# SebastianBitsch/SRGAN-ST

Measured on AMD Instinct MI355X. Metric: HR images/sec (96px x4, B=16/GPU) G+D+ST-loss step, higher is better.
Workload: dtype f32; 1 GPU; srgan_x4_hr96_b16_G+D+ST-loss step: adv+mse+st, D updated every step (train.py:116-164; BASELINE metric); global_batch=16, hr=96, lr=24, parallelism=dp1, hip_graph=True, d_update_interval=1, d_sr_forward=run: all three discriminator forwards of train.py:136,155,158

## Files before the change

### include/srganst.h

```cpp
#ifndef SRGANST_H
#define SRGANST_H
#include <stdint.h>
#ifdef __cplusplus
extern "C" {
#endif

const char* sst_last_error(void);
int sst_version(void);
const char* sst_arch(void);
int sst_clear_error(void);
int sst_reload_env(void);

int sst_st_loss_workspace(int B, int H, int W, int64_t* partial_floats);
int sst_st_loss_fwd(const float* sr, const float* gt, float* loss, float* gS, float* partials,
                    unsigned* counter, int B, int H, int W, float sigma, float rho, int normalize,
                    void* stream);
int sst_st_loss_bwd(const float* sr, const float* gS, float* dsr, const float* scale_dev,
                    float scale_host, int accumulate, int B, int H, int W, float sigma, float rho,
                    void* stream);
int sst_st_maps_workspace(int B, int H, int W, int64_t* tile_floats);
int sst_st_maps(const float* x, const float* gt, float* Sx, float* Sgt, float* Fx, float* Fgt, float* d, float* tile_sums,
                int B, int H, int W, float sigma, float rho, int normalize, void* stream);
int sst_st_pixel_loss_fwd(const float* sr, const float* gt, float* loss, float* gS, float* partials, unsigned* counter,
                          float* pix_loss, float* pix_partials, int pix_mode, int B, int H, int W, float sigma, float rho,
// ... 106 lines not shown
int sst_conv_fwd_resin(const float* x, const float* y2, const float* ones, const float* bn_scale, const float* bn_shift,
                       float* h_out, const float* wp, float* y, const float* bias, float* stats, float* stats_cnt,
                       int B, int H, int W, int Cin, int Cout, int ksize, void* stream);
int sst_conv_dgrad_fused(const float* g, const float* y2, const float* cA, const float* cB, const float* cC,
                         const float* in_scale, const float* in_shift, const float* in_slope, float in_slope_const,
                         int in_act, float* dy_out, const float* wp, float* out, const float* residual,
                         const float* epi_y, const float* epi_scale, const float* epi_shift, const float* epi_slope,
                         float epi_slope_const, int epi_act, float* epi_partial, int B, int H, int W, int Cin, int Cout,
                         int ksize, void* stream);
int sst_conv_wgrad_chunks2(int B, int H, int W, int Cin, int Cout, int ksize, int stride, int njobs);
int sst_conv_wgrad_groups_ok(int B, int H, int W, int Cin, int Cout, int ksize, int stride, int grp_images);
int sst_conv_wgrad_grp(const float* x, const float* dy, float* slab, float* dw, const float* in_scale,
                   const float* in_shift, const float* in_slope, float in_slope_const, int in_act,
                   int B, int H, int W, int Cin, int Cout, int stride, int ksize, int accumulate,
                       int grp_images, void* stream);
int sst_conv_wgrad_pending_reduce(int B, int H, int W, int Cin, int Cout, int ksize, int stride, int has_in_scale, int in_act);
int sst_wgrad_reduce_multi(const void* jobs, int njobs, void* stream);
int sst_wgrad_c3_supported(int C, int ksize);
int64_t sst_wgrad_c3_slab_floats(int B, int H, int W, int C);
int sst_wgrad_c3(const float* big, const float* small, float* slab, float* dw, const float* in_slope,
                 float in_slope_const, int in_act, int kind, int B, int H, int W, int C, int accumulate,
                 void* stream);

int64_t sst_conv9_c3_packed_floats(int Cout_eff);
int sst_conv9_c3_pack(const float* w, float* wp, int Cout, int Cin, int mode, void* stream);
int sst_conv9_c3_fwd(const float* x, const float* wp, float* y, const float* bias, int B, int H, int W,
                     int Cout, void* stream);
int64_t sst_conv9_to3_packed_floats(int C);
int sst_conv9_to3_pack(const float* w, float* wp, int C, void* stream);
int sst_conv9_to3_fwd(const float* x, const float* wp, float* y, float* y_pre, const float* bias,
// ... 151 lines not shown
```

### srgan-st_amd/csrc/bn_elem.hip

```cpp
#include "common.h"
#include <cstdlib>

typedef float f32x4 __attribute__((ext_vector_type(4)));

namespace {

constexpr int NT = 256;

__global__ __launch_bounds__(NT) void bn_finalize_kernel(const float* __restrict__ stats, const float* __restrict__ cnt,
                                                         int ntiles, int C, const float* __restrict__ gamma,
                                                         const float* __restrict__ beta, float* __restrict__ run_mean,
                                                         float* __restrict__ run_var, float* __restrict__ mean_out,
                                                         float* __restrict__ rstd_out, float* __restrict__ scale,
                                                         float* __restrict__ shift, float eps, float momentum, int groups) {
  __shared__ float red[2][NT / 64];
  const int c = blockIdx.x;
  for (int grp = 0; grp < groups; ++grp, stats += (size_t)ntiles * 2 * C, cnt += ntiles, mean_out += C, rstd_out += C, scale += C,
           shift += C) {
  constexpr int KT = 4;
  float ts[KT], tm[KT], tn[KT];
  float s = 0.f, n = 0.f;
#pragma unroll
  for (int k = 0; k < KT; ++k) {
    const int t = threadIdx.x + k * NT;
// ... 426 lines not shown
      if (scale) {
        ksc = *reinterpret_cast<const f32x4*>(scale + c);
        ksh = *reinterpret_cast<const f32x4*>(shift + c);
      }
      if (cA) {
        kA = *reinterpret_cast<const f32x4*>(cA + c);
        kB = *reinterpret_cast<const f32x4*>(cB + c);
        kC = *reinterpret_cast<const f32x4*>(cC + c);
      }
    }
#pragma unroll
    for (int j = 0; j < 4; ++j) {
      float gz = gv[j];
      if (act) {
        const float z = scale ? fmaf(yv[j], ksc[j], ksh[j]) : yv[j];
        gz = z > 0.f ? gz : gz * slope;
      }
      o[j] = cA ? fmaf(kA[j], gz, fmaf(kB[j], yv[j], kC[j])) : gz;
    }
    if (uW == 0) {
      reinterpret_cast<f32x4*>(dy)[i] = o;
    } else {
      const int64_t r = i / c4n;
      const int X = (int)(r % uW);
      const int64_t t = r / uW;
      const int Y = (int)(t % uH);
      const int64_t b = t / uH;
      float* d = dy + (((b * (uH >> 1) + (Y >> 1)) * (uW >> 1) + (X >> 1)) * (int64_t)(4 * C)) + 2 * (Y & 1) + (X & 1);
#pragma unroll
      for (int j = 0; j < 4; ++j) d[4 * (c + j)] = o[j];
    }
// ... 248 lines not shown
```

### srgan-st_amd/csrc/common.h

```cpp
#pragma once
#include <hip/hip_runtime.h>
#include <cstdarg>
#include <cstdio>
#include <cstdint>

#define SST_API extern "C" __attribute__((visibility("default")))

enum : int {
  SST_OK = 0,
  SST_ERR_ARG = -1,
  SST_ERR_UNSUPPORTED = -2,
  SST_ERR_HIP = -3,
};

int sst_set_error(int code, const char* fmt, ...);

#define SST_REQUIRE(cond, ...)                                   \
  do {                                                           \
    if (!(cond)) return sst_set_error(SST_ERR_ARG, __VA_ARGS__); \
  } while (0)

#define SST_LAUNCH_CHECK(name)                                                                   \
  do {                                                                                           \
    hipError_t e_ = hipGetLastError();                                                           \
    if (e_ != hipSuccess) return sst_set_error(SST_ERR_HIP, "%s: %s", name, hipGetErrorString(e_)); \
  } while (0)

const char* sst_env(const char* name);

static inline hipStream_t sst_stream(void* s) { return reinterpret_cast<hipStream_t>(s); }

__device__ __forceinline__ float wave_sum(float v) {
#pragma unroll
  for (int o = 32; o > 0; o >>= 1) v += __shfl_xor(v, o, 64);
  return v;
}

template <int NT>
__device__ __forceinline__ float block_sum(float v, float* red) {
  v = wave_sum(v);
  const int wid = threadIdx.x >> 6, lane = threadIdx.x & 63;
  __syncthreads();
  if (lane == 0) red[wid] = v;
  __syncthreads();
  float t = 0.f;
// ... 83 lines not shown
```

### srgan-st_amd/csrc/conv_fwd.hip

```cpp
#include "conv_common.h"
#include <cstdlib>
#include "conv_epilogue.h"

int sst_launch_conv_fwd2(const Conv3Args& a, int stride, hipStream_t st);
int sst_launch_conv_band(const Conv3Args& a, int R, hipStream_t st, const BandAcc* acc);
int sst_conv_band_rows(int B, int H, int W, int Cin, int Cout, int ksize, int stride);

namespace {

constexpr int BIG_MIN_TILES = 2048;
inline bool use_big_tiles(const Conv3Args& a, int ksize) {
  if (ksize != 3 || a.Cout < 64 || a.in2 || a.side_out) return false;
  if (a.out_mode != OUT_NHWC && a.out_mode != OUT_SHUFFLE && a.out_mode != OUT_STRIDE2) return false;
  if (const char* e = sst_env("SST_CONV_BIG")) return atoi(e) != 0;
  const long tiles = (long)a.B * ((a.Ho + 7) / 8) * ((a.Wo + 7) / 8) * ((a.Cout + 63) / 64);
  return tiles >= BIG_MIN_TILES;
}

template <int KS, int S>
__device__ __forceinline__ void conv_fwd_body(const Conv3Args& a, const int bx, const int by) {
  const int KK = a.ksy * a.ksx;
  constexpr int PW = (TWO - 1) * S + KS, PH = (THO - 1) * S + KS, NP = PW * PH;
  constexpr int LDS_FLOATS = (NP * LDSC > 4 * 32 * 33) ? NP * LDSC : 4 * 32 * 33;
  __shared__ __attribute__((aligned(16))) float lds[LDS_FLOATS];
// ... 454 lines not shown
        if (bias) v += *reinterpret_cast<const f32x4*>(bias + c);
        *reinterpret_cast<f32x4*>(ps + li * C3F_OST + c) = v;
      }
    const int b = t / (H * tpr), rem = t - b * (H * tpr);
    const int oy = rem / tpr, x0 = (rem - oy * tpr) << 5;
    float* const yp = y + (((size_t)b * H + oy) * W + x0) * Cout;
#pragma unroll
    for (int i = 0; i < 8; ++i) {
      const int idx = lane + 64 * i, px = idx >> 4, c4 = (idx & 15) * 4;
      *reinterpret_cast<f32x4*>(yp + (size_t)px * Cout + c4) = *reinterpret_cast<const f32x4*>(ps + px * C3F_OST + c4);
    }
  }
}

typedef float f32x4c __attribute__((ext_vector_type(4)));
__global__ __launch_bounds__(CONV_NT) void conv3_to3_kernel(const float* __restrict__ x, const float* __restrict__ wp,
                                                            float* __restrict__ y, int B, int H, int W, int nmt, int nsp) {
  extern __shared__ __attribute__((aligned(16))) float pl_all[];
  const int wave = __builtin_amdgcn_readfirstlane(threadIdx.x >> 6), lane = threadIdx.x & 63;
  const int seg = blockIdx.x * 4 + wave;
  if (seg >= B * H * nsp) return;
  const int row = seg / nsp, Ws = W / nsp, xb = (seg - row * nsp) * Ws;
  const int b = row / H, oy = row - b * H;
  const int lm = lane & 15, lg = lane >> 4;
  float* const pl = pl_all + (size_t)wave * nmt * 16 * 12;
  float bw[3][4][4];
  {
    const int tx = lm / 3, ci = lm - tx * 3;
#pragma unroll
    for (int ty = 0; ty < 3; ++ty)
#pragma unroll
      for (int q = 0; q < 4; ++q)
#pragma unroll
        for (int t = 0; t < 4; ++t) {
          const int co = 16 * q + 4 * lg + t, tap = ty * 3 + tx;
          bw[ty][q][t] = lm < 9 ? wp[(size_t)(tap * 8 + (co >> 3)) * 256 + (((co & 7) >> 2) * 32 + ci) * 4 + (co & 3)] : 0.f;
        }
  }
  auto load_tile = [&](int mt, f32x4c (&a)[3][4]) {
    const int xp = xb + mt * 16 + lm - 1;
#pragma unroll
    for (int ty = 0; ty < 3; ++ty) {
      const int iy = oy - 1 + ty;
      const bool ok = (unsigned)iy < (unsigned)H && (unsigned)xp < (unsigned)W;
      const float* src = x + (((size_t)b * H + (ok ? iy : 0)) * W + (ok ? xp : 0)) * 64 + 4 * lg;
#pragma unroll
      for (int q = 0; q < 4; ++q) {
        const f32x4c v = *reinterpret_cast<const f32x4c*>(src + 16 * q);
        a[ty][q] = ok ? v : f32x4c{0.f, 0.f, 0.f, 0.f};
      }
    }
  };
  f32x4c ac[3][4], an[3][4];
  load_tile(0, ac);
  for (int mt = 0; mt < nmt; ++mt) {
    if (mt + 1 < nmt) load_tile(mt + 1, an);
    f32x4c acc = {0.f, 0.f, 0.f, 0.f};
#pragma unroll
    for (int ty = 0; ty < 3; ++ty)
#pragma unroll
      for (int q = 0; q < 4; ++q)
#pragma unroll
        for (int t = 0; t < 4; ++t) acc = __builtin_amdgcn_mfma_f32_16x16x4f32(ac[ty][q][t], bw[ty][q][t], acc, 0, 0, 0);
    if (lm < 9) {
#pragma unroll
      for (int r = 0; r < 4; ++r) pl[(mt * 16 + 4 * lg + r) * 12 + lm] = acc[r];
    }
#pragma unroll
    for (int ty = 0; ty < 3; ++ty)
#pragma unroll
      for (int q = 0; q < 4; ++q) ac[ty][q] = an[ty][q];
  }
  float* const out = y + (((size_t)b * H + oy) * W + xb) * 3;
  for (int i = lane; i < 3 * Ws; i += 64) {
    const int xo = i / 3, ci = i - xo * 3;
    out[i] = (pl[xo * 12 + ci] + pl[(xo + 1) * 12 + 3 + ci]) + pl[(xo + 2) * 12 + 6 + ci];
  }
}

__global__ void pack_conv_kernel(const float* __restrict__ w, float* __restrict__ wp, int Cout, int Cin, int KK,
                                 int mode, int64_t total) {
  const int O = mode ? Cin : Cout, I = mode ? Cout : Cin;
  const int ncb = (I + 63) / 64;
  const int64_t base = packed_floats_base(O, I, KK);
  for (int64_t idx = blockIdx.x * (int64_t)blockDim.x + threadIdx.x; idx < total; idx += (int64_t)gridDim.x * blockDim.x) {
    if (idx >= base) {
      const int64_t q = idx - base;
      const int l = (q >> 2) & 63, tap = (q >> 10) % 9;
      const int o = (int)((q >> 10) / 9) * 16 + (l & 15), i = ((q >> 8) & 3) * 16 + (l >> 4) * 4 + (q & 3);
      wp[idx] = mode == 0 ? w[((size_t)o * Cin + i) * KK + tap] : w[((size_t)i * Cin + o) * KK + (KK - 1 - tap)];
      continue;
    }
// ... 365 lines not shown
  Conv3Args a{};
  conv_shape_args(a, B, H, W, Cin, Cout, ksize, stride);
  a.out_mode = out_mode;
  a.in2 = fused_in ? reinterpret_cast<const float*>(1) : nullptr;
  return conv_fwd_select(a, ksize, stride, 0).name;
}

SST_API int sst_conv_fwd(const float* x, const float* wp, float* y, float* y_pre, const float* bias, const float* in_scale,
                         const float* in_shift, const float* in_slope, float in_slope_const, int in_act,
                         const float* residual, float* stats, float* stats_cnt, int out_mode, int B, int H, int W, int Cin,
                         int Cout, int ksize, int stride, void* stream) {
  return conv_fwd_impl(x, wp, y, y_pre, bias, in_scale, in_shift, in_slope, in_slope_const, in_act, residual, stats, stats_cnt,
                       out_mode, B, H, W, Cin, Cout, ksize, stride, nullptr, nullptr, nullptr, nullptr, 0.f, 0, nullptr, stream);
}

SST_API int sst_conv_dgrad_bwdstats(const float* x, const float* wp, float* y, const float* residual, const float* epi_y,
                                    const float* epi_scale, const float* epi_shift, const float* epi_slope,
                                    float epi_slope_const, int epi_act, float* epi_partial, int B, int H, int W, int Cin,
                                    int Cout, int ksize, void* stream) {
  SST_REQUIRE(epi_y && epi_partial, "sst_conv_dgrad_bwdstats: epi_y / epi_partial");
  return conv_fwd_impl(x, wp, y, nullptr, nullptr, nullptr, nullptr, nullptr, 0.f, ACT_NONE, residual, nullptr, nullptr, OUT_NHWC,
                       B, H, W, Cin, Cout, ksize, 1, epi_y, epi_scale, epi_shift, epi_slope, epi_slope_const, epi_act, epi_partial,
                       stream);
}

SST_API int sst_conv_dgrad_fused(const float* g, const float* y2, const float* cA, const float* cB, const float* cC,
                                 const float* in_scale, const float* in_shift, const float* in_slope, float in_slope_const,
                                 int in_act, float* dy_out, const float* wp, float* out, const float* residual,
                                 const float* epi_y, const float* epi_scale, const float* epi_shift, const float* epi_slope,
                                 float epi_slope_const, int epi_act, float* epi_partial, int B, int H, int W, int Cin, int Cout,
// ... 200 lines not shown
```

### srgan-st_amd/csrc/conv_wgrad.hip

```cpp
#include "conv_common.h"
#include <cstring>
#include <cstdlib>

namespace {

constexpr int SUB = 64;
constexpr int WLD = 64 + 4;

struct WgJob {
  const float* x; const float* dy; float* slab; float* dw;
  const float* in_scale; const float* in_shift; const float* in_slope;
  float in_slope_const; int in_act;
};

constexpr int WG_TAB_MAX = 40;
struct WgJobTab { WgJob j[WG_TAB_MAX]; };

struct WgradArgs {
  int grouped;
  int nchunk;
  const float* x;
  const float* dy;
  float* slab;
  const float* in_scale;
// ... 366 lines not shown
    __syncthreads();
    if (pl == 0 && cob + co < Cout) {
      float* out = slab + (size_t)blockIdx.x * 9 * Cout * 3;
#pragma unroll
      for (int k = 0; k < 27; ++k) {
        const float t = ((acc[k] + red[0][co][k]) + red[1][co][k]) + red[2][co][k];
        const int ky = k / 9, kx = (k % 9) / 3, ci = k % 3;
        out[((size_t)(ky * 3 + kx) * Cout + cob + co) * 3 + ci] = t;
      }
    }
  }
}
constexpr int C3M_ROW = 104;
constexpr int C3M_WAVE = 3 * C3M_ROW + 96;
constexpr int C3M_TPW = 4;
__global__ __launch_bounds__(CONV_NT) void wgrad_k3c3_mfma_kernel(const float* __restrict__ x, const float* __restrict__ dy,
                                                                  float* __restrict__ slab, int B, int H, int W, int ntiles) {
  __shared__ float patch[4 * C3M_WAVE];
  __shared__ float scr[4 * 32 * 33];
  const int tid = threadIdx.x, wave = __builtin_amdgcn_readfirstlane(tid >> 6), lane = tid & 63;
  const int li = lane & 31, lh = lane >> 5;
  constexpr int Cout = 64;
  float* const ps = patch + wave * C3M_WAVE;
  const int tpr = W >> 5;
  const int ky = li / 9, kr = li - ky * 9;
  const float* const bl = ps + (li < 27 ? ky * C3M_ROW + kr + 3 * lh : 3 * C3M_ROW);
  f32x16 acc[2];
#pragma unroll
  for (int h = 0; h < 2; ++h)
#pragma unroll
    for (int r = 0; r < 16; ++r) acc[h][r] = 0.f;
  for (int i = lane; i < 96; i += 64) ps[3 * C3M_ROW + i] = 0.f;
  float av[2][16][2], xv[2][5];
  auto issue = [&](int it, float (&a_)[16][2], float (&x_)[5]) {
    const int t = (blockIdx.x * C3M_TPW + it) * 4 + wave;
    const bool live = it < C3M_TPW && t < ntiles;
    const int b = t / (H * tpr), rem = t - b * (H * tpr);
    const int y = rem / tpr, x0 = (rem - y * tpr) << 5;
    const float* dp = dy + (live ? (((size_t)b * H + y) * W + x0 + lh) * Cout + li : 0);
#pragma unroll
    for (int ks = 0; ks < 16; ++ks) {
      a_[ks][0] = live ? dp[(size_t)(2 * ks) * Cout] : 0.f;
      a_[ks][1] = live ? dp[(size_t)(2 * ks) * Cout + 32] : 0.f;
    }
#pragma unroll
    for (int u = 0; u < 5; ++u) {
      const int i = lane + 64 * u;
      const int r = i / 102, c = i - r * 102;
      const int iy = y - 1 + r, fx = (x0 - 1) * 3 + c;
      const bool ok = live && i < 306 && (unsigned)iy < (unsigned)H && (unsigned)fx < (unsigned)(W * 3);
      x_[u] = ok ? x[((size_t)b * H + iy) * W * 3 + fx] : 0.f;
    }
  };
  issue(0, av[0], xv[0]);
#pragma unroll
  for (int it = 0; it < C3M_TPW; ++it) {
#pragma unroll
    for (int u = 0; u < 5; ++u) {
      const int i = lane + 64 * u;
      if (i < 306) ps[(i / 102) * C3M_ROW + i % 102] = xv[it & 1][u];
    }
    if (it + 1 < C3M_TPW) issue(it + 1, av[(it + 1) & 1], xv[(it + 1) & 1]);
#pragma unroll
    for (int ks = 0; ks < 16; ++ks) {
      const float bv = bl[6 * ks];
      acc[0] = __builtin_amdgcn_mfma_f32_32x32x2f32(av[it & 1][ks][0], bv, acc[0], 0, 0, 0);
      acc[1] = __builtin_amdgcn_mfma_f32_32x32x2f32(av[it & 1][ks][1], bv, acc[1], 0, 0, 0);
    }
  }
  float* const out = slab + (size_t)blockIdx.x * 9 * Cout * 3;
#pragma unroll
  for (int h = 0; h < 2; ++h) {
    __syncthreads();
#pragma unroll
    for (int r = 0; r < 16; ++r) scr[(wave * 32 + (r & 3) + 8 * (r >> 2) + 4 * lh) * 33 + li] = acc[h][r];
    __syncthreads();
#pragma unroll
    for (int j = 0; j < 4; ++j) {
      const int row = 8 * wave + 4 * lh + j;
      const float v = ((scr[row * 33 + li] + scr[(32 + row) * 33 + li]) + scr[(64 + row) * 33 + li]) + scr[(96 + row) * 33 + li];
      if (li < 27) out[((size_t)(li / 3) * Cout + 32 * h + row) * 3 + li % 3] = v;
    }
  }
}
constexpr int C3R_OUT = 16, C3R_GRP = 1024 / C3R_OUT;
__global__ __launch_bounds__(1024) void c3m_reduce_kernel(const float* __restrict__ slab, float* __restrict__ dw, int nchunk,
                                                          int accumulate) {
  __shared__ float part[C3R_GRP][C3R_OUT + 1];
  constexpr int TOTAL = 9 * 64 * 3;
  const int o = threadIdx.x & (C3R_OUT - 1), gq = threadIdx.x / C3R_OUT;
  const int i = blockIdx.x * C3R_OUT + o;
  float t = 0.f;
  int c = gq;
  for (; c + 7 * C3R_GRP < nchunk; c += 8 * C3R_GRP) {
    float v[8];
#pragma unroll
    for (int u = 0; u < 8; ++u) v[u] = slab[(size_t)(c + C3R_GRP * u) * TOTAL + i];
#pragma unroll
    for (int u = 0; u < 8; ++u) t += v[u];
  }
  {
    float v[8];
#pragma unroll
    for (int u = 0; u < 8; ++u) v[u] = c + C3R_GRP * u < nchunk ? slab[(size_t)(c + C3R_GRP * u) * TOTAL + i] : 0.f;
#pragma unroll
    for (int u = 0; u < 8; ++u) t += v[u];
  }
  part[gq][o] = t;
  __syncthreads();
  if (threadIdx.x < 64) {
    const int oo = threadIdx.x & (C3R_OUT - 1), q = threadIdx.x / C3R_OUT;
    t = 0.f;
#pragma unroll
    for (int k = 0; k < C3R_GRP / 4; ++k) t += part[q * (C3R_GRP / 4) + k][oo];
    t += __shfl_xor(t, 16, 64);
    t += __shfl_xor(t, 32, 64);
    if (q == 0) {
      const int ii = blockIdx.x * C3R_OUT + oo;
      const int tap = ii / 192, oc = ii - tap * 192;
      float* d = dw + (size_t)oc * 9 + tap;
      *d = accumulate ? *d + t : t;
    }
  }
}
inline bool k3c3_mfma_applies(int W, int Cout) { return (W & 31) == 0 && Cout == 64 && !sst_env("SST_WGRAD_NO_K3C3_MFMA"); }
inline int k3c3_mfma_chunks(int B, int H, int W) { return (B * H * (W >> 5) + 4 * C3M_TPW - 1) / (4 * C3M_TPW); }

inline bool k3c3_applies(int Cin, int ksize, int stride, bool has_in_scale, int in_act) {
  return Cin == 3 && ksize == 3 && stride == 1 && !has_in_scale && in_act == ACT_NONE;
}

struct WgBandPlan { int R, bpc, nchunk, nbands; size_t lds; };
inline WgBandPlan wgrad_band_plan(int B, int H, int W, int Cin, int Cout, int ksize, int stride, int njobs) {
  WgBandPlan best{0, 0, 0, 0, 0};
  if (ksize != 3 || stride != 1 || (Cin & 63) || (Cout & 63) || (W & 3) || W < 4) return best;
  if (const char* e = sst_env("SST_WGRAD_BAND")) {
    if (atoi(e) == 0) return best;
  }
// ... 576 lines not shown
      s2.B = B; s2.H = H; s2.W = W; s2.Cin = Cin; s2.Cout = Cout; s2.Ho = a.Ho; s2.Wo = a.Wo;
      s2.dbg = sst_env("SST_WGRAD_S2_DBG") ? atoi(sst_env("SST_WGRAD_S2_DBG")) : 0;
      s2.dw = pl.pending ? nullptr : dw;
      s2.accumulate = accumulate & 1;
      s2.gB = grouped ? grp_images : 0;
      s2.tiles_x = a.Wo / p2.tw; s2.tiles_img = (a.Ho / p2.th) * s2.tiles_x; s2.ntiles = p2.ntiles; s2.tpc = p2.tpc;
      int rc;
      if (stride == 2) rc = p2.tw == 8 ? launch_wgrad_s2_t<2, 2, 8, 8>(s2, p2, st) : launch_wgrad_s2_t<2, 2, 6, 8>(s2, p2, st);
      else rc = p2.tw == 8 ? launch_wgrad_s2_t<1, 4, 8, 8>(s2, p2, st) : launch_wgrad_s2_t<1, 4, 6, 8>(s2, p2, st);
      if (rc != SST_OK) return rc;
      break;
    }
    case WgKind::K3C3_MFMA:
      wgrad_k3c3_mfma_kernel<<<pl.nchunk, CONV_NT, 0, st>>>(x, dy, slab, B, H, W, B * H * (W >> 5));
      SST_LAUNCH_CHECK("wgrad_k3c3_mfma_kernel");
      c3m_reduce_kernel<<<9 * 64 * 3 / C3R_OUT, 1024, 0, st>>>(slab, dw, pl.nchunk, accumulate & 1);
      SST_LAUNCH_CHECK("c3m_reduce_kernel");
      return SST_OK;
    case WgKind::K3C3: {
      const size_t lds = (size_t)(C3_ROWS + 2) * ((W + 2) * 3 + 3) * sizeof(float);
      SST_REQUIRE(lds <= 48 * 1024, "sst_conv_wgrad: image too wide for the 3-channel-input kernel (W=%d)", W);
      wgrad_k3c3_kernel<<<dim3(pl.nchunk, 1), CONV_NT, lds, st>>>(x, dy, slab, B, H, W, Cout);
      break;
    }
    case WgKind::GENERAL_VEC: conv_wgrad_kernel<true><<<grid, CONV_NT, 0, st>>>(a, no_tab); break;
    case WgKind::GENERAL_SCALAR: conv_wgrad_kernel<false><<<grid, CONV_NT, 0, st>>>(a, no_tab); break;
  }
  SST_LAUNCH_CHECK(pl.name);
  if (pl.pending == 0 || (accumulate & 4)) return SST_OK;
  launch_wgrad_reduce(slab, dw, pl.nchunk, KK, Cout, Cin, accumulate, nullptr, 1, st);
  SST_LAUNCH_CHECK("wgrad_reduce_kernel");
  return SST_OK;
}

SST_API int sst_wgrad_reduce_multi(const void* jobs, int njobs, void* stream) {
  static_assert(sizeof(WrJob) == 40, "WrJob layout");
  SST_REQUIRE(jobs && njobs > 0 && njobs <= WR_TAB_MAX, "sst_wgrad_reduce_multi: 1..%d jobs", WR_TAB_MAX);
  WrJobTab tab{};
  memcpy(tab.j, jobs, (size_t)njobs * sizeof(WrJob));
  int maxb = 0;
  for (int i = 0; i < njobs; ++i) {
    WrJob& j = tab.j[i];
    SST_REQUIRE(j.slab && j.dw && j.nchunk > 0 && j.KK > 0 && j.Cout > 0 && j.Cin > 0, "sst_wgrad_reduce_multi: bad job %d", i);
    const int64_t total = (int64_t)j.KK * j.Cout * j.Cin;
    if ((j.Cin & 3) == 0 && j.nchunk >= 8) {
      j.blocks = (int)((total / 4 + 63) / 64);
// ... 42 lines not shown
```

### srgan-st_amd/srganst/_abi.py

```python
from __future__ import annotations

import ctypes
import os
from ctypes import c_char_p, c_float, c_int, c_int64, c_void_p, POINTER

_HERE = os.path.dirname(os.path.abspath(__file__))
LIB_PATH = os.environ.get("SST_LIB_PATH") or os.path.join(_HERE, "lib", "libsrganst.so")

P = c_void_p

SIGNATURES = {
    "sst_last_error": (c_char_p, []),
    "sst_version": (c_int, []),
    "sst_arch": (c_char_p, []),
    "sst_clear_error": (c_int, []),
    "sst_reload_env": (c_int, []),
    "sst_st_loss_workspace": (c_int, [c_int, c_int, c_int, POINTER(c_int64)]),
    "sst_st_loss_fwd": (c_int, [P, P, P, P, P, P, c_int, c_int, c_int, c_float, c_float, c_int, P]),
    "sst_st_loss_bwd": (c_int, [P, P, P, P, c_float, c_int, c_int, c_int, c_int, c_float, c_float, P]),
    "sst_st_pixel_loss_fwd": (c_int, [P, P, P, P, P, P, P, P, c_int, c_int, c_int, c_int, c_float, c_float, c_int, P]),
    "sst_st_pixel_loss_bwd": (c_int, [P, P, P, P, P, c_float, c_float, c_int, c_int, c_int, c_int, c_int, c_float, c_float, P]),
    "sst_st_maps_workspace": (c_int, [c_int, c_int, c_int, POINTER(c_int64)]),
    "sst_st_maps": (c_int, [P, P, P, P, P, P, P, P, c_int, c_int, c_int, c_float, c_float, c_int, P]),
    "sst_st_route": (c_int, [c_float, c_float, POINTER(c_int), POINTER(c_int)]),
# ... 61 lines not shown
                                 c_int, c_int, c_int, c_int, c_int, c_int, c_int, P]),
    "sst_conv_dgrad_fused_acc": (c_int, [P, P, P, P, P, c_float, c_int, P, P, P, P, P, P, P, P, c_float, c_int, P, P, P, P, c_float, P, P, P,
                                         P, c_int, c_int, c_int, c_int, c_int, c_int, c_int, P]),
    "sst_bn_finalize_acc": (c_int, [P, c_int, c_int, c_float, P, P, P, P, P, P, P, P, c_float, c_float, P]),
    "sst_conv_fwd_resin": (c_int, [P, P, P, P, P, P, P, P, P, P, P, c_int, c_int, c_int, c_int, c_int, c_int, P]),
    "sst_conv_dgrad_bwdstats": (c_int, [P, P, P, P, P, P, P, P, c_float, c_int, P, c_int, c_int, c_int, c_int, c_int, c_int, P]),
    "sst_conv_dgrad_fused": (c_int, [P, P, P, P, P, P, P, P, c_float, c_int, P, P, P, P, P, P, P, P, c_float, c_int, P,
                                     c_int, c_int, c_int, c_int, c_int, c_int, P]),
    "sst_conv_wgrad_chunks2": (c_int, [c_int, c_int, c_int, c_int, c_int, c_int, c_int, c_int]),
    "sst_conv_wgrad_groups_ok": (c_int, [c_int, c_int, c_int, c_int, c_int, c_int, c_int, c_int]),
    "sst_conv_wgrad_grp": (c_int, [P, P, P, P, P, P, P, c_float, c_int, c_int, c_int, c_int, c_int, c_int,
                                   c_int, c_int, c_int, c_int, P]),
    "sst_conv_wgrad_grouped": (c_int, [P, c_int, c_int, c_int, c_int, c_int, c_int, c_int, c_int, c_int, P]),
    "sst_conv_wgrad_pending_reduce": (c_int, [c_int, c_int, c_int, c_int, c_int, c_int, c_int, c_int, c_int]),
    "sst_wgrad_reduce_multi": (c_int, [P, c_int, P]),
    "sst_bn_finalize_grp": (c_int, [P, P, c_int, c_int, c_int, P, P, P, P, P, P, P, P, c_float, c_float, P]),
    "sst_bn_eval_affine": (c_int, [P, P, P, P, P, P, c_int, c_float, P]),
    "sst_bn_residual": (c_int, [P, P, P, P, P, P, c_int64, c_int, P]),
    "sst_bwd_reduce_blocks": (c_int, [c_int64, c_int]),
    "sst_bwd_finalize": (c_int, [P, c_int, c_int, c_float, P, P, P, P, P, P, P, P, P, c_int, P]),
    "sst_bwd_reduce_grp": (c_int, [P, P, P, P, P, P, c_float, c_int, P, c_int64, c_int, c_int, P]),
    "sst_bwd_finalize_grp": (c_int, [P, c_int, c_int, c_float, c_int, P, P, P, P, P, P, P, P, c_int, P]),
    "sst_bwd_apply_grp": (c_int, [P, P, P, P, P, P, c_float, c_int, P, P, P, P, c_int64, c_int, c_int, P]),
    "sst_bwd_finalize_wide": (c_int, [P, c_int, c_int, c_float, P, P, P, P, P, P, P, P, P, c_int, P, P, P]),
    "sst_act_bwd_partial_blocks": (c_int, [c_int64]),
    "sst_act_bwd_partial": (c_int, [P, P, P, P, c_float, P, P, c_int64, c_int, c_int, c_int, P]),
    "sst_bwd_apply": (c_int, [P, P, P, P, P, P, c_float, c_int, P, P, P, P, c_int64, c_int, c_int, c_int, P]),
    "sst_add": (c_int, [P, P, P, c_int64, P]),
    "sst_transpose": (c_int, [P, P, c_int, c_int, c_int, c_int, c_int, P]),
    "sst_transpose_affine": (c_int, [P, P, c_int, c_int, c_int, c_int, c_int, P, P, P]),
# ... 110 lines not shown
```

### srgan-st_amd/srganst/disc_graph.py

```python
from __future__ import annotations

from collections import namedtuple
from dataclasses import dataclass

import torch

from . import ops
from ._state import KeptPass, state
from .ops import ACT_SLOPE

LRELU = 0.2

PLAN = [(0, None, 1), (2, 3, 2), (5, 6, 1), (8, 9, 2), (11, 12, 1), (14, 15, 2), (17, 18, 1), (20, 21, 2)]


class _Layer:
    __slots__ = ("ci", "bi", "stride", "y", "mean", "rstd", "scale", "shift", "st", "cnt")

    def __init__(self, ci, bi, stride, y, mean=None, rstd=None, scale=None, shift=None):
        self.ci, self.bi, self.stride, self.y = ci, bi, stride, y
        self.mean, self.rstd, self.scale, self.shift, self.st, self.cnt = mean, rstd, scale, shift, None, None

    def epi(self, prefix=""):
        return {prefix + "y": self.y, prefix + "scale": self.scale, prefix + "shift": self.shift, prefix + "slope_const": LRELU,
# ... 187 lines not shown
            ops.linear_wgrad(dh1, sv.flat, dw0, db0, accumulate=acc)
    B, H, W, C = sv.layers[-1].y.shape
    sink.g = ops.linear_dgrad(dh1, p["classifier.0.weight"], nhwc=(C, H * W)).view(B, H, W, C)
    return sink


def _bn_act_bwd(part, g, n, **kw):
    return ops.bwd_finalize_apply(part, g, n=n, **kw) if part is not None else ops.bwd_reduce_apply(g, n=n, **kw)


def backward_features(module, p, sv, sink, need_param_grads, need_dx, defer_wgrad=None, defer_below=None):
    wg, acc, g = need_param_grads, sink.acc, sink.g
    groups, gB = sv.groups, sv.gB
    dx = part = None
    reduces = [] if ops.WGRAD_REDUCE_MULTI else None
    for li in reversed(range(len(sv.layers))):
        r, below = sv.layers[li], sv.layers[li - 1] if li > 0 else None
        x, in_kw = sv.input_of(li)
        n = r.y.numel() // r.y.shape[-1] // groups
        wname = f"features.{r.ci}.weight"
        cin = p[wname].shape[1]
        if r.bi is not None:
            gam = p[f"features.{r.bi}.weight"]
            dg = sink.take(f"features.{r.bi}.weight") if wg else torch.empty_like(gam)
            db = sink.take(f"features.{r.bi}.bias") if wg else torch.empty_like(gam)
            dy = _bn_act_bwd(part, g, n, **r.epi(), mean=r.mean, rstd=r.rstd, gamma=gam, dgamma=dg, dbeta=db, accumulate=acc and wg,
                             groups=groups)
        elif wg:
            dy = _bn_act_bwd(part, g, n, **r.epi(), dbeta=sink.take(f"features.{r.ci}.bias"), accumulate=acc, groups=groups)
        else:
            dy = ops.bwd_apply(g, **r.epi(), groups=groups)
        part = None
        if wg:
            dwc = sink.take(wname)

            def launch(x=x, dy=dy, dwc=dwc, stride=r.stride, in_kw=in_kw, red=None):
                ops.conv_wgrad(x, dy, dwc, 3, stride, **in_kw, accumulate=acc, grp=gB, defer_reduce=red)
            if defer_wgrad is not None and (defer_below is None or li < defer_below):
                ev = torch.cuda.Event()
                ev.record()
                defer_wgrad.append((ev, launch, (x, dy, dwc, in_kw["in_scale"], in_kw["in_shift"])))
            else:
                with ops.SideStream(x, dy, dwc):
                    launch(red=reduces)
        if li == 0 and not need_dx:
            break
        if r.stride == 1:
            if below is not None:
                g, part = ops.conv_dgrad_bwdstats(dy, sv.wd[wname], cin, 3, **below.epi("epi_"), grp=gB)
            else:
                g = ops.conv_fwd(dy, sv.wd[wname], cin, 3, 1)[0]
        else:
            epi = below.epi() if below is not None and (below.bi is not None or wg) else None
            out = ops.conv_s2_dgrad(dy, sv.ws2[wname], x.shape[1], x.shape[2], cin, epi=epi, grp=gB)
            g, part = out if epi is not None else (out, None)
        if li == 0:
            dx = ops.transpose(g, to_nchw=True)
    if reduces:
        with ops.SideStream(*[t for j in reduces for t in j[:2]]):
            ops.wgrad_reduce_flush(reduces)
    ops.join_side()
    return sink.grads(), dx


def backward(module, p, sv, dout, need_param_grads, need_dx):
    sink = backward_classifier(module, p, sv, dout, need_param_grads)
    return backward_features(module, p, sv, sink, need_param_grads, need_dx)

# ... 28 lines not shown
```

### srgan-st_amd/srganst/ops.py

```python
from __future__ import annotations

import ctypes
import os

import torch

from . import _abi
from ._abi import check, ptr, stream_ptr
from ._state import state

OUT_NHWC, OUT_SHUFFLE, OUT_NCHW_CLAMP, OUT_UNSHUFFLE = 0, 1, 2, 3
ACT_NONE, ACT_SLOPE = 0, 1
BN_EPS, BN_MOMENTUM = 1e-5, 0.1


TRACE = None

TRACE_HBM = None


def _launch(fn, args, what, flops, name_fn, keep):
    check(fn(*args, stream_ptr()), what)
    if TRACE is not None:
        TRACE.setdefault(name_fn(), []).append((lambda: fn(*args, stream_ptr()), flops, keep))
# ... 235 lines not shown
    if defer_reduce is not None and TRACE is None:
        pend = _abi.lib().sst_conv_wgrad_pending_reduce(B, H, W, cin, cout, ksize, stride, int(in_scale is not None), int(in_act))
        if pend:
            assert dw_out.is_contiguous()
            defer_reduce.append((slab, dw_out, pend, ksize * ksize, cout, cin, int(bool(accumulate))))
    inp, ikeep = _in_args(in_scale, in_shift, in_slope, in_slope_const, in_act)
    args = (ptr(x), ptr(dy), ptr(slab), ptr(dw_out), *inp, B, H, W, cin, cout, stride, ksize, int(bool(accumulate)) | (4 if pend else 0),
            int(grp))

    def name():
        n = _wgrad_name(B, H, W, cin, cout, ksize, stride, 1)
        return n + ("+c3m_reduce_kernel" if n == "wgrad_k3c3_mfma_kernel" else "+wgrad_reduce_kernel")
    _launch(_abi.lib().sst_conv_wgrad_grp, args, "sst_conv_wgrad", 2.0 * B * ho * wo * cout * cin * ksize * ksize, name,
            (x, dy, slab, dw_out, *ikeep))
    return dw_out


WGRAD_REDUCE_MULTI = os.environ.get("SST_WGRAD_REDUCE_MULTI", "1") != "0"


def wgrad_reduce_flush(jobs):
    import ctypes
    import struct
    while jobs:
        js, jobs[:] = jobs[:24], jobs[24:]
        buf = b"".join(struct.pack("<QQiiiiii", slab.data_ptr(), dw.data_ptr(), nch, kk, cout, cin, acc, 0)
                       for slab, dw, nch, kk, cout, cin, acc in js)
        check(_abi.lib().sst_wgrad_reduce_multi(ctypes.c_char_p(buf), len(js), stream_ptr()), "sst_wgrad_reduce_multi")


# ... 715 lines not shown
```

Before: 3258 HR images/s.

## Fuse LeakyReLU backward into discriminator first-layer wgrad and dgrad kernels

```diff
diff --git a/include/srganst.h b/include/srganst.h
--- a/include/srganst.h
+++ b/include/srganst.h
@@ -144,6 +144,13 @@
                    const float* in_shift, const float* in_slope, float in_slope_const, int in_act,
                    int B, int H, int W, int Cin, int Cout, int stride, int ksize, int accumulate,
                        int grp_images, void* stream);
+int sst_conv_wgrad_k3c3_act_supported(int B, int H, int W, int Cout);
+int64_t sst_conv_wgrad_k3c3_act_slab_floats(int B, int H, int W);
+int sst_conv_wgrad_k3c3_act(const float* x3, const float* g, const float* y, float slope_const, float* dw, float* db,
+                            float* slab, int B, int H, int W, int accumulate, void* stream);
+int sst_conv3_to3_act_supported(int B, int H, int W);
+int sst_conv3_to3_act(const float* g, const float* y, float slope_const, const float* wp, float* dx, int B, int H, int W,
+                      void* stream);
 int sst_conv_wgrad_pending_reduce(int B, int H, int W, int Cin, int Cout, int ksize, int stride, int has_in_scale, int in_act);
 int sst_wgrad_reduce_multi(const void* jobs, int njobs, void* stream);
 int sst_wgrad_c3_supported(int C, int ksize);
diff --git a/srgan-st_amd/csrc/bn_elem.hip b/srgan-st_amd/csrc/bn_elem.hip
--- a/srgan-st_amd/csrc/bn_elem.hip
+++ b/srgan-st_amd/csrc/bn_elem.hip
@@ -464,7 +464,7 @@
       float gz = gv[j];
       if (act) {
         const float z = scale ? fmaf(yv[j], ksc[j], ksh[j]) : yv[j];
-        gz = z > 0.f ? gz : gz * slope;
+        gz = sst_act_bwd(gz, z, slope);
       }
       o[j] = cA ? fmaf(kA[j], gz, fmaf(kB[j], yv[j], kC[j])) : gz;
     }
diff --git a/srgan-st_amd/csrc/common.h b/srgan-st_amd/csrc/common.h
--- a/srgan-st_amd/csrc/common.h
+++ b/srgan-st_amd/csrc/common.h
@@ -29,6 +29,8 @@
 const char* sst_env(const char* name);
 
 static inline hipStream_t sst_stream(void* s) { return reinterpret_cast<hipStream_t>(s); }
+
+__device__ inline float sst_act_bwd(float gz, float z, float slope) { return z > 0.f ? gz : gz * slope; }
 
 __device__ __forceinline__ float wave_sum(float v) {
 #pragma unroll
diff --git a/srgan-st_amd/csrc/conv_fwd.hip b/srgan-st_amd/csrc/conv_fwd.hip
--- a/srgan-st_amd/csrc/conv_fwd.hip
+++ b/srgan-st_amd/csrc/conv_fwd.hip
@@ -492,8 +492,9 @@
 }
 
 typedef float f32x4c __attribute__((ext_vector_type(4)));
-__global__ __launch_bounds__(CONV_NT) void conv3_to3_kernel(const float* __restrict__ x, const float* __restrict__ wp,
-                                                            float* __restrict__ y, int B, int H, int W, int nmt, int nsp) {
+template <bool ACT>
+__device__ __forceinline__ void conv3_to3_body(const float* __restrict__ x, const float* __restrict__ wp, float* __restrict__ y, int B,
+                                               int H, int W, int nmt, int nsp, const float* __restrict__ act_y, float slope) {
   extern __shared__ __attribute__((aligned(16))) float pl_all[];
   const int wave = __builtin_amdgcn_readfirstlane(threadIdx.x >> 6), lane = threadIdx.x & 63;
   const int seg = blockIdx.x * 4 + wave;
@@ -515,22 +516,46 @@
           bw[ty][q][t] = lm < 9 ? wp[(size_t)(tap * 8 + (co >> 3)) * 256 + (((co & 7) >> 2) * 32 + ci) * 4 + (co & 3)] : 0.f;
         }
   }
+  f32x4c yn[3][4];
   auto load_tile = [&](int mt, f32x4c (&a)[3][4]) {
     const int xp = xb + mt * 16 + lm - 1;
 #pragma unroll
     for (int ty = 0; ty < 3; ++ty) {
       const int iy = oy - 1 + ty;
       const bool ok = (unsigned)iy < (unsigned)H && (unsigned)xp < (unsigned)W;
-      const float* src = x + (((size_t)b * H + (ok ? iy : 0)) * W + (ok ? xp : 0)) * 64 + 4 * lg;
+      const size_t off = (((size_t)b * H + (ok ? iy : 0)) * W + (ok ? xp : 0)) * 64 + 4 * lg;
+      const float* src = x + off;
 #pragma unroll
       for (int q = 0; q < 4; ++q) {
         const f32x4c v = *reinterpret_cast<const f32x4c*>(src + 16 * q);
         a[ty][q] = ok ? v : f32x4c{0.f, 0.f, 0.f, 0.f};
       }
-    }
+      if constexpr (ACT) {
+#pragma unroll
+        for (int q = 0; q < 4; ++q) yn[ty][q] = *reinterpret_cast<const f32x4c*>(act_y + off + 16 * q);
+      }
+    }
+  };
+  auto take = [&](f32x4c (&dst)[3][4], const f32x4c (&src)[3][4]) {
+#pragma unroll
+    for (int ty = 0; ty < 3; ++ty)
+#pragma unroll
+      for (int q = 0; q < 4; ++q) {
+        if constexpr (ACT) {
+#pragma unroll
+          for (int t = 0; t < 4; ++t) dst[ty][q][t] = sst_act_bwd(src[ty][q][t], yn[ty][q][t], slope);
+        } else {
+          dst[ty][q] = src[ty][q];
+        }
+      }
   };
   f32x4c ac[3][4], an[3][4];
-  load_tile(0, ac);
+  if constexpr (ACT) {
+    load_tile(0, an);
+    take(ac, an);
+  } else {
+    load_tile(0, ac);
+  }
   for (int mt = 0; mt < nmt; ++mt) {
     if (mt + 1 < nmt) load_tile(mt + 1, an);
     f32x4c acc = {0.f, 0.f, 0.f, 0.f};
@@ -544,16 +569,22 @@
 #pragma unroll
       for (int r = 0; r < 4; ++r) pl[(mt * 16 + 4 * lg + r) * 12 + lm] = acc[r];
     }
-#pragma unroll
-    for (int ty = 0; ty < 3; ++ty)
-#pragma unroll
-      for (int q = 0; q < 4; ++q) ac[ty][q] = an[ty][q];
+    take(ac, an);
   }
   float* const out = y + (((size_t)b * H + oy) * W + xb) * 3;
   for (int i = lane; i < 3 * Ws; i += 64) {
     const int xo = i / 3, ci = i - xo * 3;
     out[i] = (pl[xo * 12 + ci] + pl[(xo + 1) * 12 + 3 + ci]) + pl[(xo + 2) * 12 + 6 + ci];
   }
+}
+__global__ __launch_bounds__(CONV_NT) void conv3_to3_kernel(const float* __restrict__ x, const float* __restrict__ wp,
+                                                            float* __restrict__ y, int B, int H, int W, int nmt, int nsp) {
+  conv3_to3_body<false>(x, wp, y, B, H, W, nmt, nsp, nullptr, 0.f);
+}
+__global__ __launch_bounds__(CONV_NT) void conv3_to3_act_kernel(const float* __restrict__ g, const float* __restrict__ act_y,
+                                                                float slope, const float* __restrict__ wp, float* __restrict__ dx,
+                                                                int B, int H, int W, int nmt, int nsp) {
+  conv3_to3_body<true>(g, wp, dx, B, H, W, nmt, nsp, act_y, slope);
 }
 
 __global__ void pack_conv_kernel(const float* __restrict__ w, float* __restrict__ wp, int Cout, int Cin, int KK,
@@ -949,6 +980,29 @@
                        out_mode, B, H, W, Cin, Cout, ksize, stride, nullptr, nullptr, nullptr, nullptr, 0.f, 0, nullptr, stream);
 }
 
+namespace {
+FwdSel conv3_to3_act_select(int B, int H, int W) {
+  Conv3Args a{};
+  conv_shape_args(a, B, H, W, 64, 3, 3, 1);
+  a.out_mode = OUT_NHWC;
+  return conv_fwd_select(a, 3, 1, 0);
+}
+}
+SST_API int sst_conv3_to3_act_supported(int B, int H, int W) {
+  if (B <= 0 || H <= 0 || W <= 0 || (int64_t)B * H * W >= (1ll << 29) || sst_env("SST_D0_UNFUSED")) return 0;
+  return conv3_to3_act_select(B, H, W).kind == FwdKind::TO3;
+}
+SST_API int sst_conv3_to3_act(const float* g, const float* y, float slope_const, const float* wp, float* dx, int B, int H, int W,
+                              void* stream) {
+  SST_REQUIRE(g && y && wp && dx, "sst_conv3_to3_act: null pointer");
+  SST_REQUIRE(sst_conv3_to3_act_supported(B, H, W), "sst_conv3_to3_act: shape not taken (B=%d H=%d W=%d)", B, H, W);
+  const FwdSel s = conv3_to3_act_select(B, H, W);
+  conv3_to3_act_kernel<<<(unsigned)((B * H * s.nsp + 3) / 4), CONV_NT, s.lds, sst_stream(stream)>>>(g, y, slope_const, wp, dx, B, H, W,
+                                                                                                    s.nmt, s.nsp);
+  SST_LAUNCH_CHECK("conv3_to3_act_kernel");
+  return SST_OK;
+}
+
 SST_API int sst_conv_dgrad_bwdstats(const float* x, const float* wp, float* y, const float* residual, const float* epi_y,
                                     const float* epi_scale, const float* epi_shift, const float* epi_slope,
                                     float epi_slope_const, int epi_act, float* epi_partial, int B, int H, int W, int Cin,
diff --git a/srgan-st_amd/csrc/conv_wgrad.hip b/srgan-st_amd/csrc/conv_wgrad.hip
--- a/srgan-st_amd/csrc/conv_wgrad.hip
+++ b/srgan-st_amd/csrc/conv_wgrad.hip
@@ -404,8 +404,10 @@
 constexpr int C3M_ROW = 104;
 constexpr int C3M_WAVE = 3 * C3M_ROW + 96;
 constexpr int C3M_TPW = 4;
-__global__ __launch_bounds__(CONV_NT) void wgrad_k3c3_mfma_kernel(const float* __restrict__ x, const float* __restrict__ dy,
-                                                                  float* __restrict__ slab, int B, int H, int W, int ntiles) {
+template <bool ACT>
+__device__ __forceinline__ void wgrad_k3c3_mfma_body(const float* __restrict__ x, const float* __restrict__ dy,
+                                                     float* __restrict__ slab, int B, int H, int W, int ntiles,
+                                                     const float* __restrict__ act_y, float slope, float* __restrict__ db_slab) {
   __shared__ float patch[4 * C3M_WAVE];
   __shared__ float scr[4 * 32 * 33];
   const int tid = threadIdx.x, wave = __builtin_amdgcn_readfirstlane(tid >> 6), lane = tid & 63;
@@ -421,17 +423,29 @@
 #pragma unroll
     for (int r = 0; r < 16; ++r) acc[h][r] = 0.f;
   for (int i = lane; i < 96; i += 64) ps[3 * C3M_ROW + i] = 0.f;
-  float av[2][16][2], xv[2][5];
+  float av[2][16][2], yv[16][2], xv[2][5], dbs[2] = {0.f, 0.f};
   auto issue = [&](int it, float (&a_)[16][2], float (&x_)[5]) {
     const int t = (blockIdx.x * C3M_TPW + it) * 4 + wave;
     const bool live = it < C3M_TPW && t < ntiles;
     const int b = t / (H * tpr), rem = t - b * (H * tpr);
     const int y = rem / tpr, x0 = (rem - y * tpr) << 5;
-    const float* dp = dy + (live ? (((size_t)b * H + y) * W + x0 + lh) * Cout + li : 0);
-#pragma unroll
-    for (int ks = 0; ks < 16; ++ks) {
-      a_[ks][0] = live ? dp[(size_t)(2 * ks) * Cout] : 0.f;
-      a_[ks][1] = live ? dp[(size_t)(2 * ks) * Cout + 32] : 0.f;
+    const size_t doff = live ? (((size_t)b * H + y) * W + x0 + lh) * Cout + li : 0;
+    const float* dp = dy + doff;
+    if constexpr (!ACT) {
+#pragma unroll
+      for (int ks = 0; ks < 16; ++ks) {
+        a_[ks][0] = live ? dp[(size_t)(2 * ks) * Cout] : 0.f;
+        a_[ks][1] = live ? dp[(size_t)(2 * ks) * Cout + 32] : 0.f;
+      }
+    } else {
+      const float* yp = act_y + doff;
+#pragma unroll
+      for (int ks = 0; ks < 16; ++ks) {
+        a_[ks][0] = dp[(size_t)(2 * ks) * Cout];
+        a_[ks][1] = dp[(size_t)(2 * ks) * Cout + 32];
+        yv[ks][0] = yp[(size_t)(2 * ks) * Cout];
+        yv[ks][1] = yp[(size_t)(2 * ks) * Cout + 32];
+      }
     }
 #pragma unroll
     for (int u = 0; u < 5; ++u) {
@@ -442,20 +456,47 @@
       x_[u] = ok ? x[((size_t)b * H + iy) * W * 3 + fx] : 0.f;
     }
   };
-  issue(0, av[0], xv[0]);
-#pragma unroll
-  for (int it = 0; it < C3M_TPW; ++it) {
+  auto stage_patch = [&](const float (&x_)[5]) {
 #pragma unroll
     for (int u = 0; u < 5; ++u) {
       const int i = lane + 64 * u;
-      if (i < 306) ps[(i / 102) * C3M_ROW + i % 102] = xv[it & 1][u];
-    }
-    if (it + 1 < C3M_TPW) issue(it + 1, av[(it + 1) & 1], xv[(it + 1) & 1]);
+      if (i < 306) ps[(i / 102) * C3M_ROW + i % 102] = x_[u];
+    }
+  };
+  auto multiply = [&](const float (&a_)[16][2]) {
 #pragma unroll
     for (int ks = 0; ks < 16; ++ks) {
       const float bv = bl[6 * ks];
-      acc[0] = __builtin_amdgcn_mfma_f32_32x32x2f32(av[it & 1][ks][0], bv, acc[0], 0, 0, 0);
-      acc[1] = __builtin_amdgcn_mfma_f32_32x32x2f32(av[it & 1][ks][1], bv, acc[1], 0, 0, 0);
+      acc[0] = __builtin_amdgcn_mfma_f32_32x32x2f32(a_[ks][0], bv, acc[0], 0, 0, 0);
+      acc[1] = __builtin_amdgcn_mfma_f32_32x32x2f32(a_[ks][1], bv, acc[1], 0, 0, 0);
+    }
+  };
+  issue(0, av[0], xv[0]);
+  if constexpr (!ACT) {
+#pragma unroll
+    for (int it = 0; it < C3M_TPW; ++it) {
+      stage_patch(xv[it & 1]);
+      if (it + 1 < C3M_TPW) issue(it + 1, av[(it + 1) & 1], xv[(it + 1) & 1]);
+      multiply(av[it & 1]);
+    }
+  } else {
+#pragma unroll 1
+    for (int it = 0; it < C3M_TPW; ++it) {
+      stage_patch(xv[0]);
+      const bool live = (blockIdx.x * C3M_TPW + it) * 4 + wave < ntiles;
+#pragma unroll
+      for (int ks = 0; ks < 16; ++ks)
+#pragma unroll
+        for (int h = 0; h < 2; ++h) {
+          float v = live ? sst_act_bwd(av[0][ks][h], yv[ks][h], slope) : 0.f;
+          asm volatile("" : "+v"(v) : : "memory");
+          av[1][ks][h] = v;
+          dbs[h] += v;
+        }
+      __builtin_amdgcn_sched_barrier(0);
+      if (it + 1 < C3M_TPW) issue(it + 1, av[0], xv[0]);
+      __builtin_amdgcn_sched_barrier(0);
+      multiply(av[1]);
     }
   }
   float* const out = slab + (size_t)blockIdx.x * 9 * Cout * 3;
@@ -472,15 +513,36 @@
       if (li < 27) out[((size_t)(li / 3) * Cout + 32 * h + row) * 3 + li % 3] = v;
     }
   }
+  if constexpr (ACT) {
+    __syncthreads();
+    scr[(wave * 2 + lh) * 64 + li] = dbs[0];
+    scr[(wave * 2 + lh) * 64 + 32 + li] = dbs[1];
+    __syncthreads();
+    if (tid < 64) {
+      float w4[4];
+#pragma unroll
+      for (int w = 0; w < 4; ++w) w4[w] = scr[(2 * w) * 64 + tid] + scr[(2 * w + 1) * 64 + tid];
+      db_slab[(size_t)blockIdx.x * 64 + tid] = ((w4[0] + w4[1]) + w4[2]) + w4[3];
+    }
+  }
+}
+__global__ __launch_bounds__(CONV_NT) void wgrad_k3c3_mfma_kernel(const float* __restrict__ x, const float* __restrict__ dy,
+                                                                  float* __restrict__ slab, int B, int H, int W, int ntiles) {
+  wgrad_k3c3_mfma_body<false>(x, dy, slab, B, H, W, ntiles, nullptr, 0.f, nullptr);
+}
+__global__ __launch_bounds__(CONV_NT) void wgrad_k3c3_mfma_act_kernel(const float* __restrict__ x, const float* __restrict__ g,
+                                                                      const float* __restrict__ act_y, float slope,
+                                                                      float* __restrict__ slab, float* __restrict__ db_slab, int B,
+                                                                      int H, int W, int ntiles) {
+  wgrad_k3c3_mfma_body<true>(x, g, slab, B, H, W, ntiles, act_y, slope, db_slab);
 }
 constexpr int C3R_OUT = 16, C3R_GRP = 1024 / C3R_OUT;
-__global__ __launch_bounds__(1024) void c3m_reduce_kernel(const float* __restrict__ slab, float* __restrict__ dw, int nchunk,
-                                                          int accumulate) {
+template <int TOTAL>
+__device__ __forceinline__ bool c3m_reduce_sum(const float* __restrict__ slab, int nchunk, int blk, int& ii, float& t) {
   __shared__ float part[C3R_GRP][C3R_OUT + 1];
-  constexpr int TOTAL = 9 * 64 * 3;
   const int o = threadIdx.x & (C3R_OUT - 1), gq = threadIdx.x / C3R_OUT;
-  const int i = blockIdx.x * C3R_OUT + o;
-  float t = 0.f;
+  const int i = blk * C3R_OUT + o;
+  t = 0.f;
   int c = gq;
   for (; c + 7 * C3R_GRP < nchunk; c += 8 * C3R_GRP) {
     float v[8];
@@ -498,20 +560,40 @@
   }
   part[gq][o] = t;
   __syncthreads();
-  if (threadIdx.x < 64) {
-    const int oo = threadIdx.x & (C3R_OUT - 1), q = threadIdx.x / C3R_OUT;
-    t = 0.f;
-#pragma unroll
-    for (int k = 0; k < C3R_GRP / 4; ++k) t += part[q * (C3R_GRP / 4) + k][oo];
-    t += __shfl_xor(t, 16, 64);
-    t += __shfl_xor(t, 32, 64);
-    if (q == 0) {
-      const int ii = blockIdx.x * C3R_OUT + oo;
-      const int tap = ii / 192, oc = ii - tap * 192;
-      float* d = dw + (size_t)oc * 9 + tap;
-      *d = accumulate ? *d + t : t;
-    }
-  }
+  if (threadIdx.x >= 64) return false;
+  const int oo = threadIdx.x & (C3R_OUT - 1), q = threadIdx.x / C3R_OUT;
+  t = 0.f;
+#pragma unroll
+  for (int k = 0; k < C3R_GRP / 4; ++k) t += part[q * (C3R_GRP / 4) + k][oo];
+  t += __shfl_xor(t, 16, 64);
+  t += __shfl_xor(t, 32, 64);
+  ii = blk * C3R_OUT + oo;
+  return q == 0;
+}
+__device__ __forceinline__ void c3m_reduce_dw(const float* __restrict__ slab, float* __restrict__ dw, int nchunk, int accumulate, int blk) {
+  int ii;
+  float t;
+  if (c3m_reduce_sum<9 * 64 * 3>(slab, nchunk, blk, ii, t)) {
+    const int tap = ii / 192, oc = ii - tap * 192;
+    float* d = dw + (size_t)oc * 9 + tap;
+    *d = accumulate ? *d + t : t;
+  }
+}
+__global__ __launch_bounds__(1024) void c3m_reduce_kernel(const float* __restrict__ slab, float* __restrict__ dw, int nchunk,
+                                                          int accumulate) {
+  c3m_reduce_dw(slab, dw, nchunk, accumulate, blockIdx.x);
+}
+constexpr int C3R_DW_WGS = 9 * 64 * 3 / C3R_OUT;
+__global__ __launch_bounds__(1024) void c3m_reduce_db_kernel(const float* __restrict__ slab, float* __restrict__ dw,
+                                                             const float* __restrict__ db_slab, float* __restrict__ db, int nchunk,
+                                                             int accumulate) {
+  if (blockIdx.x < C3R_DW_WGS) {
+    c3m_reduce_dw(slab, dw, nchunk, accumulate, blockIdx.x);
+    return;
+  }
+  int ii;
+  float t;
+  if (c3m_reduce_sum<64>(db_slab, nchunk, blockIdx.x - C3R_DW_WGS, ii, t)) db[ii] = accumulate ? db[ii] + t : t;
 }
 inline bool k3c3_mfma_applies(int W, int Cout) { return (W & 31) == 0 && Cout == 64 && !sst_env("SST_WGRAD_NO_K3C3_MFMA"); }
 inline int k3c3_mfma_chunks(int B, int H, int W) { return (B * H * (W >> 5) + 4 * C3M_TPW - 1) / (4 * C3M_TPW); }
@@ -1118,7 +1200,7 @@
     case WgKind::K3C3_MFMA:
       wgrad_k3c3_mfma_kernel<<<pl.nchunk, CONV_NT, 0, st>>>(x, dy, slab, B, H, W, B * H * (W >> 5));
       SST_LAUNCH_CHECK("wgrad_k3c3_mfma_kernel");
-      c3m_reduce_kernel<<<9 * 64 * 3 / C3R_OUT, 1024, 0, st>>>(slab, dw, pl.nchunk, accumulate & 1);
+      c3m_reduce_kernel<<<C3R_DW_WGS, 1024, 0, st>>>(slab, dw, pl.nchunk, accumulate & 1);
       SST_LAUNCH_CHECK("c3m_reduce_kernel");
       return SST_OK;
     case WgKind::K3C3: {
@@ -1134,6 +1216,28 @@
   if (pl.pending == 0 || (accumulate & 4)) return SST_OK;
   launch_wgrad_reduce(slab, dw, pl.nchunk, KK, Cout, Cin, accumulate, nullptr, 1, st);
   SST_LAUNCH_CHECK("wgrad_reduce_kernel");
+  return SST_OK;
+}
+
+SST_API int sst_conv_wgrad_k3c3_act_supported(int B, int H, int W, int Cout) {
+  if (B <= 0 || H <= 0 || W <= 0 || Cout <= 0 || sst_env("SST_D0_UNFUSED")) return 0;
+  return wgrad_plan(B, H, W, 3, Cout, 3, 1, 1, false, ACT_NONE, false).kind == WgKind::K3C3_MFMA;
+}
+SST_API int64_t sst_conv_wgrad_k3c3_act_slab_floats(int B, int H, int W) {
+  return (int64_t)k3c3_mfma_chunks(B, H, W) * (9 * 64 * 3 + 64);
+}
+SST_API int sst_conv_wgrad_k3c3_act(const float* x3, const float* g, const float* y, float slope_const, float* dw, float* db,
+                                    float* slab, int B, int H, int W, int accumulate, void* stream) {
+  SST_REQUIRE(x3 && g && y && dw && db && slab, "sst_conv_wgrad_k3c3_act: null pointer");
+  SST_REQUIRE(sst_conv_wgrad_k3c3_act_supported(B, H, W, 64), "sst_conv_wgrad_k3c3_act: shape not taken (B=%d H=%d W=%d)", B, H, W);
+  SST_REQUIRE((int64_t)B * H * W < (1ll << 31), "sst_conv_wgrad_k3c3_act: too many pixels");
+  const int nchunk = k3c3_mfma_chunks(B, H, W);
+  float* const db_slab = slab + (size_t)nchunk * 9 * 64 * 3;
+  hipStream_t st = sst_stream(stream);
+  wgrad_k3c3_mfma_act_kernel<<<nchunk, CONV_NT, 0, st>>>(x3, g, y, slope_const, slab, db_slab, B, H, W, B * H * (W >> 5));
+  SST_LAUNCH_CHECK("wgrad_k3c3_mfma_act_kernel");
+  c3m_reduce_db_kernel<<<C3R_DW_WGS + 64 / C3R_OUT, 1024, 0, st>>>(slab, dw, db_slab, db, nchunk, accumulate & 1);
+  SST_LAUNCH_CHECK("c3m_reduce_db_kernel");
   return SST_OK;
 }
 
diff --git a/srgan-st_amd/srganst/_abi.py b/srgan-st_amd/srganst/_abi.py
--- a/srgan-st_amd/srganst/_abi.py
+++ b/srgan-st_amd/srganst/_abi.py
@@ -99,6 +99,11 @@
     "sst_conv_wgrad_grouped": (c_int, [P, c_int, c_int, c_int, c_int, c_int, c_int, c_int, c_int, c_int, P]),
     "sst_conv_wgrad_pending_reduce": (c_int, [c_int, c_int, c_int, c_int, c_int, c_int, c_int, c_int, c_int]),
     "sst_wgrad_reduce_multi": (c_int, [P, c_int, P]),
+    "sst_conv_wgrad_k3c3_act_supported": (c_int, [c_int, c_int, c_int, c_int]),
+    "sst_conv_wgrad_k3c3_act_slab_floats": (c_int64, [c_int, c_int, c_int]),
+    "sst_conv_wgrad_k3c3_act": (c_int, [P, P, P, c_float, P, P, P, c_int, c_int, c_int, c_int, P]),
+    "sst_conv3_to3_act_supported": (c_int, [c_int, c_int, c_int]),
+    "sst_conv3_to3_act": (c_int, [P, P, c_float, P, P, c_int, c_int, c_int, P]),
     "sst_bn_finalize_grp": (c_int, [P, P, c_int, c_int, c_int, P, P, P, P, P, P, P, P, c_float, c_float, P]),
     "sst_bn_eval_affine": (c_int, [P, P, P, P, P, P, c_int, c_float, P]),
     "sst_bn_residual": (c_int, [P, P, P, P, P, P, c_int64, c_int, P]),
diff --git a/srgan-st_amd/srganst/disc_graph.py b/srgan-st_amd/srganst/disc_graph.py
--- a/srgan-st_amd/srganst/disc_graph.py
+++ b/srgan-st_amd/srganst/disc_graph.py
@@ -225,6 +225,9 @@
     groups, gB = sv.groups, sv.gB
     dx = part = None
     reduces = [] if ops.WGRAD_REDUCE_MULTI else None
+    r0 = sv.layers[0]
+    first_act = r0.bi is None and r0.stride == 1
+    fuse_w = wg and first_act and ops.conv_wgrad_act_supported(sv.x3, r0.y.shape[-1])
     for li in reversed(range(len(sv.layers))):
         r, below = sv.layers[li], sv.layers[li - 1] if li > 0 else None
         x, in_kw = sv.input_of(li)
@@ -237,32 +240,44 @@
             db = sink.take(f"features.{r.bi}.bias") if wg else torch.empty_like(gam)
             dy = _bn_act_bwd(part, g, n, **r.epi(), mean=r.mean, rstd=r.rstd, gamma=gam, dgamma=dg, dbeta=db, accumulate=acc and wg,
                              groups=groups)
-        elif wg:
+        elif wg and not (li == 0 and fuse_w):
             dy = _bn_act_bwd(part, g, n, **r.epi(), dbeta=sink.take(f"features.{r.ci}.bias"), accumulate=acc, groups=groups)
+        elif li == 0 and first_act and (not need_dx or ops.conv3_to3_act_supported(g)):
+            dy = None
         else:
             dy = ops.bwd_apply(g, **r.epi(), groups=groups)
         part = None
         if wg:
             dwc = sink.take(wname)
-
-            def launch(x=x, dy=dy, dwc=dwc, stride=r.stride, in_kw=in_kw, red=None):
-                ops.conv_wgrad(x, dy, dwc, 3, stride, **in_kw, accumulate=acc, grp=gB, defer_reduce=red)
+            if li == 0 and fuse_w:
+                dbc = sink.take(f"features.{r.ci}.bias")
+                held = side = (x, g, r.y, dwc, dbc)
+
+                def launch(x=x, g=g, y=r.y, dwc=dwc, dbc=dbc, red=None):
+                    ops.conv_wgrad_act(x, g, y, LRELU, dwc, dbc, accumulate=acc)
+            else:
+                held, side = (x, dy, dwc, in_kw["in_scale"], in_kw["in_shift"]), (x, dy, dwc)
+
+                def launch(x=x, dy=dy, dwc=dwc, stride=r.stride, in_kw=in_kw, red=None):
+                    ops.conv_wgrad(x, dy, dwc, 3, stride, **in_kw, accumulate=acc, grp=gB, defer_reduce=red)
             if defer_wgrad is not None and (defer_below is None or li < defer_below):
                 ev = torch.cuda.Event()
                 ev.record()
-                defer_wgrad.append((ev, launch, (x, dy, dwc, in_kw["in_scale"], in_kw["in_shift"])))
+                defer_wgrad.append((ev, launch, held))
             else:
-                with ops.SideStream(x, dy, dwc):
+                with ops.SideStream(*side):
                     launch(red=reduces)
         if li == 0 and not need_dx:
             break
         if r.stride == 1:
             if below is not None:
                 g, part = ops.conv_dgrad_bwdstats(dy, sv.wd[wname], cin, 3, **below.epi("epi_"), grp=gB)
+            elif dy is None:
+                g = ops.conv3_to3_act(g, r.y, LRELU, sv.wd[wname])
             else:
                 g = ops.conv_fwd(dy, sv.wd[wname], cin, 3, 1)[0]
         else:
-            epi = below.epi() if below is not None and (below.bi is not None or wg) else None
+            epi = below.epi() if below is not None and (below.bi is not None or (wg and not (li == 1 and fuse_w))) else None
             out = ops.conv_s2_dgrad(dy, sv.ws2[wname], x.shape[1], x.shape[2], cin, epi=epi, grp=gB)
             g, part = out if epi is not None else (out, None)
         if li == 0:
diff --git a/srgan-st_amd/srganst/ops.py b/srgan-st_amd/srganst/ops.py
--- a/srgan-st_amd/srganst/ops.py
+++ b/srgan-st_amd/srganst/ops.py
@@ -273,6 +273,35 @@
     _launch(_abi.lib().sst_conv_wgrad_grp, args, "sst_conv_wgrad", 2.0 * B * ho * wo * cout * cin * ksize * ksize, name,
             (x, dy, slab, dw_out, *ikeep))
     return dw_out
+
+
+def conv_wgrad_act_supported(x3, cout):
+    B, H, W, cin = x3.shape
+    return cin == 3 and bool(_abi.lib().sst_conv_wgrad_k3c3_act_supported(B, H, W, int(cout)))
+
+
+def conv_wgrad_act(x3, g, y, slope_const, dw_out, db_out, accumulate=False):
+    B, H, W, _ = x3.shape
+    assert tuple(g.shape) == tuple(y.shape) == (B, H, W, 64) and tuple(dw_out.shape) == (64, 3, 3, 3) and db_out.numel() == 64
+    slab = _f32(_abi.lib().sst_conv_wgrad_k3c3_act_slab_floats(B, H, W), like=x3)
+    args = (ptr(x3), ptr(g), ptr(y), float(slope_const), ptr(dw_out), ptr(db_out), ptr(slab), B, H, W, int(bool(accumulate)))
+    _launch(_abi.lib().sst_conv_wgrad_k3c3_act, args, "sst_conv_wgrad_k3c3_act", 2.0 * B * H * W * 64 * 3 * 9,
+            lambda: "wgrad_k3c3_mfma_kernel+c3m_reduce_kernel", (x3, g, y, dw_out, db_out, slab))
+    return dw_out, db_out
+
+
+def conv3_to3_act_supported(g):
+    B, H, W, c = g.shape
+    return c == 64 and bool(_abi.lib().sst_conv3_to3_act_supported(B, H, W))
+
+
+def conv3_to3_act(g, y, slope_const, wd):
+    B, H, W, _ = g.shape
+    assert tuple(y.shape) == tuple(g.shape)
+    dx = _f32(B, H, W, 3, like=g)
+    _launch(_abi.lib().sst_conv3_to3_act, (ptr(g), ptr(y), float(slope_const), ptr(wd), ptr(dx), B, H, W), "sst_conv3_to3_act",
+            2.0 * B * H * W * 3 * 64 * 9, lambda: "conv3_to3_kernel", (g, y, wd, dx))
+    return dx
 
 
 WGRAD_REDUCE_MULTI = os.environ.get("SST_WGRAD_REDUCE_MULTI", "1") != "0"
```

Result: no change. 3282 HR images/s, median of 6 (+0.7%).
